# AutoGPTQ/AutoGPTQ

Measured on AMD Instinct MI355X. Metric: int4 g128 QuantLinear fwd GB/s + tokens/s, Llama-7B shapes, higher is better.
Workload: dtype f16; 1 GPU; Llama-7B linear shapes (4096->4096 x4, 4096->11008 x2, 11008->4096) x 32 blocks = 224 layers, int4 g128 no act-order, M=1 rows per step, 128 launches/step in one hipGraph (q|k|v and gate|up of a block: one gptq_forward_multi launch each); layers=224, launches=128, parallelism=single

## Files before the change

### autogptq_amd/csrc/capi.hip

```cpp
#include <stdarg.h>
#include <stdio.h>
#include <string.h>

#include <algorithm>
#include <cstdlib>
#include <vector>

#include "common.cuh"
#include "launch.h"
#include "../../include/gptq_mi355x_lab.h"

using namespace gptq;

namespace {

thread_local char g_err[512] = "";

int fail(int code, const char* fmt, ...) {
    va_list ap;
    va_start(ap, fmt);
    vsnprintf(g_err, sizeof(g_err), fmt, ap);
    va_end(ap);
    return code;
}
// ... 1687 lines not shown
    if (e != hipSuccess) return hip_fail(e, "gptq_unprepack_decode launch");
    return GPTQ_OK;
}

int gptq_permute_columns(const void* x, const int32_t* perm, int M, int K, int dtype, void* x_out, void* stream) {
    if (!x || !perm || !x_out) return fail(GPTQ_ERR_NULL, "x/perm/x_out must be non-NULL");
    if (!dtype_ok(dtype)) return fail(GPTQ_ERR_UNSUPPORTED, "unsupported dtype enum %d", dtype);
    if (M <= 0 || K <= 0) return fail(GPTQ_ERR_SHAPE, "M (%d) and K (%d) must be > 0", M, K);
    hipError_t e = launch_permute_columns(x, perm, M, K, dtype, x_out, (hipStream_t)stream);
    if (e != hipSuccess) return hip_fail(e, "gptq_permute_columns launch");
    return GPTQ_OK;
}

int gptq_describe_plan(const gptq_layer_t* L, int M, const gptq_tuning_t* tune, char* out, size_t out_bytes) {
    if (!out || out_bytes == 0) return fail(GPTQ_ERR_NULL, "out must be non-NULL");
    out[0] = 0;
    int rc = check_layer(L);
    if (rc) return rc;
    if (M <= 0) return fail(GPTQ_ERR_SHAPE, "M must be > 0, got %d", M);
    if (tune && (tune->path == 2 || tune->path == 4)) return fail(GPTQ_ERR_UNSUPPORTED, "tuning.path = %d was retired in round 6", tune->path);
    if (tiled_pair_call(L, M, tune)) {
        const gptq_layer_t* one[1] = {L};
        const TiledPlan tp = plan_tiled(one, 1, M, tune);
        snprintf(out, out_bytes, "path=gemv kernel=strips ln=4 waves=%d u=%d ksplit=%d mt=%d strips=%d pair=1 perm=0 epilogue=fused", tp.waves, tp.u, tp.ksplit, tp.mt,
                 tp.strips_total);
        return GPTQ_OK;
    }
    const bool unfused_epilogue = L->epilogue != GPTQ_EPI_NONE && !fused_epilogue_ok(L, M, tune);
    gptq_layer_t Lc = *L;
    gptq_tuning_t local;
    if (unfused_epilogue) {
        Lc.epilogue = GPTQ_EPI_NONE;
        tune = inner_tuning(L, M, tune, &local);
    }
    gptq_layer_t Pseq;
    const gptq_layer_t* one_t[1] = {&Lc};
    if (!unfused_epilogue && Lc.epilogue == GPTQ_EPI_NONE && want_tiled(one_t, 1, M, tune)) {
        const TiledPlan tp = plan_tiled(one_t, 1, M, tune);
        snprintf(out, out_bytes, "path=gemv kernel=strips ln=4 waves=%d u=%d ksplit=%d mt=%d strips=%d pair=0 perm=0 epilogue=none", tp.waves, tp.u, tp.ksplit, tp.mt,
                 tp.strips_total);
    } else if (!unfused_epilogue && want_stream_seq(L, M, tune, &Pseq)) {
        const gptq_layer_t* one[1] = {&Pseq};
        const StreamPlan sp = plan_stream(one, 1, M, nullptr);
        snprintf(out, out_bytes, "path=gemv kernel=stream ln=%d waves=%d u=%d ksplit=%d mt=%d strips=%d pair=0 perm=2 epilogue=none", sp.ln, sp.waves,
                 sp.u, sp.ksplit, sp.mt, sp.strips_total);
    } else if (want_stream(&Lc, M, tune)) {
        const gptq_layer_t* one[1] = {&Lc};
        const StreamPlan sp = plan_stream(one, 1, M, tune);
        snprintf(out, out_bytes, "path=gemv kernel=stream ln=%d waves=%d u=%d ksplit=%d mt=%d strips=%d pair=0 perm=0 epilogue=none", sp.ln, sp.waves,
                 sp.u, sp.ksplit, sp.mt, sp.strips_total);
    } else if (want_gemm(&Lc, M, tune)) {
        const GemmPlan g = plan_gemm(Lc, M, tune);
        const char* kern = g.f32 ? "f32_mfma" : g.rows ? "rows" : g.panel ? "panel" : g.wsk ? "wide_sk" : g.wide ? (g.wide_tiled ? "wide_copy" : "wide") : g.mid ? "mid" : (g.stream64 ? "stream64" : (g.strip16 ? "strip16" : (g.skinny ? "skinny64" : "tiled")));
        snprintf(out, out_bytes, "path=gemm kernel=%s mt=%d bk=%d kg=%d ksplit=%d tiles=%dx%d tail=%d tail_slices=%d perm=%d dma=%d waves=%d u=%d epilogue=%s", kern, g.mt, g.bk,
                 g.kg == 2 ? 2 : 1, g.ksplit, g.nbm, g.nbn, g.tail, g.tail ? (1 << g.tail_lg) : 1, g.use_seq ? 1 : 0, (g.glds || g.stream64 || g.mid) ? 1 : 0, g.waves, g.u,
                 unfused_epilogue ? "separate" : "none");
    } else {
        const GemvPlan v = plan_gemv(Lc, M, tune);
        const char* kern = v.mfma ? "mfma" : (v.mfmag ? "mfma_generic" : "generic");
        snprintf(out, out_bytes, "path=gemv kernel=%s ln=%d waves=%d u=%d ksplit=%d mt=%d strips=%d pair=%d perm=%d epilogue=%s%s", kern, v.ln,
                 v.waves, v.u, v.ksplit, v.mt, v.strips, v.pair ? 1 : 0, v.xperm ? 2 : (v.use_seq ? 1 : 0),
                 v.pair ? "fused" : (unfused_epilogue ? "separate" : "none"), v.magic ? " deq=magic" : "");
    }
// ... 110 lines not shown
```

### autogptq_amd/csrc/gemv_tiled.hip

```cpp
#include "gemv_tiled_kernel.cuh"

namespace gptq {

hipError_t launch_tiled_act(const TiledPlan& pl, const TiledParams& p, int dtype, hipStream_t st);
hipError_t init_gemv_tiled_act_device();
hipError_t launch_tiled_peer(const TiledPlan& pl, const TiledParams& p, int dtype, hipStream_t st);
hipError_t init_gemv_tiled_peer_device();
hipError_t launch_tiled_pair(const TiledPlan& pl, const TiledParams& p, int dtype, hipStream_t st);
hipError_t init_gemv_tiled_pair_device();
hipError_t launch_tiled_multi(const TiledPlan& pl, const TiledParams& p, int dtype, hipStream_t st);
hipError_t init_gemv_tiled_multi_device();

int tiled_max_waves(int u, int nstr) { return (u == 2 || nstr == 4) ? 16 : 8; }
static int tiled_kpl(int bits) { return bits == 8 ? 16 : 32; }
static int tiled_chunk_bytes(int bits) { return bits == 3 ? 768 : (bits == 2 ? 512 : 1024); }
static int tiled_rec_bytes(int bits) { return bits == 8 ? 64 : 48; }

static bool tiled_pair_layer(const gptq_layer_t& L) { return L.epilogue == GPTQ_EPI_SILU_MUL && L.g_idx == nullptr && L.N % (2 * GPTQ_STRIP_COLS) == 0; }

bool tiled_layer_ok(const gptq_layer_t& L) {
    if (!L.qweight_tiled || !L.qconst_tiled || L.tiled_cols != GPTQ_STRIP_COLS || (L.epilogue != GPTQ_EPI_NONE && !tiled_pair_layer(L))) return false;
    if (L.bits != 4 && L.bits != 8 && L.bits != 3 && L.bits != 2) return false;
    if (L.bits == 2 && L.epilogue != GPTQ_EPI_NONE) return false;
    if (L.g_idx != nullptr && !(L.perm && L.qweight_seq)) return false;
    if (L.dtype != GPTQ_F16 && L.dtype != GPTQ_BF16) return false;
    if (L.K % 32 || L.N % GPTQ_STRIP_COLS) return false;
    const int kpl = tiled_kpl(L.bits);
    const int gu = L.group_size / kpl;
    return L.group_size % kpl == 0 && (L.group_size >= L.K || (gu & (gu - 1)) == 0);
}

size_t tiled_weight_bytes(const gptq_layer_t& L) {
    const int cke = 4 * tiled_kpl(L.bits);
    return (size_t)((L.K + cke - 1) / cke) * tiled_chunk_bytes(L.bits) * (size_t)(L.N / GPTQ_STRIP_COLS);
}
size_t tiled_const_bytes(const gptq_layer_t& L) {
// ... 71 lines not shown
    if (tune && tune->waves && tune->reserved[0]) {
        waves = tune->waves; u = tune->reserved[0];
    } else {
        const int wgs = strips * pl.ksplit;
        if (wgs <= 256) { waves = 16; u = 2; }
        else if (wgs <= 512) { waves = 8; u = 2; }
        else { waves = 4; u = 4; }
        if (wgs <= 128 && chunks >= 64 && pl.ksplit == 1) { waves = 8; u = 4; }
        if (pl.mt > 4) { waves = 8; u = 4; }
        if (pair && waves == 4) waves = 8;
        if (pair && waves == 8 && u == 4 && (double)((chunks + 15) / 16 * 16) / chunks - (double)((chunks + 7) / 8 * 8) / chunks >= 0.1) u = 2;
        if (nstr > 1) { waves = nstr == 4 ? 16 : 8; u = 4; }
        if (nstr == 2 && pl.mt <= 2 && A.K <= 7168) waves = 4;
        if (nstr == 2 && pl.mt == 4 && waves == 8 && (double)((chunks + 15) / 16 * 16) / chunks - (double)((chunks + 7) / 8 * 8) / chunks >= 0.1) u = 2;
        if (pl.mt == 4 && waves == 4 && !pair && nstr == 1 && ((size_t)160 * 1024 / lds_need(ks, 4)) * 4 < 12) waves = 8;
        const int per = pair ? 2 : nstr;
        while (waves > per && (waves / (2 * per)) * u >= cps) waves /= 2;
    }
    if (pair && (waves & 1)) return pl;
    if (nstr > 1 && pl.mt <= 2 && (waves > 8 || u != 4)) return pl;
    if (nstr > 1 && waves % nstr != 0) return pl;
    if (waves < 1 || waves > 16 || (u != 2 && u != 4)) return pl;
    if (waves > tiled_max_waves(u, nstr)) return pl;
    pl.waves = waves;
    pl.u = u;
    pl.zm2 = A.bits == 4 && A.dtype == GPTQ_BF16 && pl.mt == 2 && (long)strips * pl.ksplit < 1024;
    pl.xstride = cps * cke * 2 + 16;
    pl.lds_bytes = lds_need(pl.ksplit, waves);
    pl.xraw_off = A.g_idx ? (int)((pl.lds_bytes - ((size_t)pl.mt * ((size_t)A.K * 2 + 16) + 16) + 15) & ~(size_t)15) : 0;
    if (pl.lds_bytes > 160 * 1024) return pl;
    pl.partial_bytes = pl.ksplit > 1 ? (size_t)(pl.ksplit - 1) * M * nsum * 8 : 0;
    pl.ok = true;
    return pl;
}

hipError_t launch_tiled(const gptq_layer_t* const* Ls, const TiledPlan& pl, const void* x, void* const* outs, int M, void* ws_header, void* ws_body,
                        hipStream_t st, const gptq_peer_group_t* pg) {
    if (!pl.ok) return hipErrorInvalidValue;
    TiledParams p{};
    if (pg) {
        if (pl.nseg != 1 || pl.mt > 4 || pg->world < 1 || pg->world > GPTQ_PEER_MAX) return hipErrorInvalidValue;
        for (int r = 0; r < pg->world; ++r) {
            p.peer.xbuf[0][r] = (char*)pg->xbuf[0][r];
            p.peer.xbuf[1][r] = (char*)pg->xbuf[1][r];
            p.peer.flags[r] = pg->flags[r];
        }
        p.peer.state = pg->state;
        p.peer.world = pg->world;
        p.peer.rank = pg->rank;
// ... 17 lines not shown
    const gptq_layer_t& A = *Ls[0];
    p.x = x;
    p.gran = (unsigned long long*)ws_body;
    p.epochs = ws_header ? (unsigned*)((char*)ws_header + WS_HEADER_EPOCH_OFFSET) : nullptr;
    p.err = ws_header ? (unsigned*)((char*)ws_header + WS_HEADER_BYTES - WS_HEADER_TAIL_BYTES) + 2 : nullptr;
#ifdef GPTQ_TILED_STAMPS
    if (pl.ksplit == 1) {
        const char* const e = getenv("GPTQ_TILED_STAMPS_PTR");
        p.gran = e ? (unsigned long long*)strtoull(e, nullptr, 0) : nullptr;
    }
#endif
    p.max_spins = 1u << 20;
    p.nseg = pl.nseg; p.M = M; p.K = A.K;
    p.chunks = pl.chunks_total; p.chunks_per_split = pl.chunks_per_split; p.ksplit = pl.ksplit;
    p.gu_shift = A.group_size >= A.K ? 26 : __builtin_ctz((unsigned)(A.group_size / tiled_kpl(A.bits)));
    p.nsum = pl.nsum;
    p.groups = pl.groups;
    p.xstride = pl.xstride;
    p.waves = pl.waves;
    p.xraw_off = pl.xraw_off;
    p.pair_strips = pl.pair ? A.N / (2 * GPTQ_STRIP_COLS) : 0;
    if (pg) {
        if (A.g_idx || A.bits == 2 || (pl.u != 2 && pl.u != 4)) return hipErrorInvalidValue;
        return launch_tiled_peer(pl, p, A.dtype, st);
    }
    if (pl.pair) return (pl.u == 2 || pl.u == 4) ? launch_tiled_pair(pl, p, A.dtype, st) : hipErrorInvalidValue;
    if (pl.nstr > 1) return (pl.u == 2 || pl.u == 4) ? launch_tiled_multi(pl, p, A.dtype, st) : hipErrorInvalidValue;
    if (A.g_idx) return launch_tiled_act(pl, p, A.dtype, st);
    return A.dtype == GPTQ_BF16 ? launch_tiled_bits<bf16, 0>(pl, p, st) : launch_tiled_bits<f16, 0>(pl, p, st);
}

hipError_t init_gemv_tiled_device() {
    hipError_t e = grant_tiled_lds<0>();
    hipError_t e2 = init_gemv_tiled_act_device();
    hipError_t e3 = init_gemv_tiled_peer_device();
    hipError_t e4 = init_gemv_tiled_pair_device();
    hipError_t e5 = init_gemv_tiled_multi_device();
    return e != hipSuccess ? e : (e2 != hipSuccess ? e2 : (e3 != hipSuccess ? e3 : (e4 != hipSuccess ? e4 : e5)));
}

}
```

### autogptq_amd/csrc/gemv_tiled_kernel.cuh

```cuda
#pragma once
#include <cstddef>

#include "gemv_shared.cuh"

namespace gptq {

struct TiledSeg {
    const void* bias;
    void* out;
    int N, col0;
};
struct PeerEpi {
    char* xbuf[2][GPTQ_PEER_MAX];
    unsigned* flags[GPTQ_PEER_MAX];
    unsigned* state;
    int world, rank;
    unsigned row_bytes, col_off_bytes, owners, pad_;
};
struct TiledParams {
    int blk_end[4];
    const void* x;
    int M, K;
    int chunks, chunks_per_split, ksplit, gu_shift, groups, xstride, waves;
    int pair_strips;
// ... 9 lines not shown
    unsigned* err;
    PeerEpi peer;
};
static_assert(offsetof(TiledParams, perm) == 128, "the entry batch of the decode-copy kernel is the first two cache lines of its arguments");

template <int BITS> struct TiledFmt;
template <> struct TiledFmt<4> { static constexpr int WPL = 4, KPL = 32, REC = 48, ZB = 1; };
template <> struct TiledFmt<8> { static constexpr int WPL = 4, KPL = 16, REC = 64, ZB = 2; };
template <> struct TiledFmt<3> { static constexpr int WPL = 3, KPL = 32, REC = 48, ZB = 1; };
template <> struct TiledFmt<2> { static constexpr int WPL = 2, KPL = 32, REC = 48, ZB = 1; };

#ifdef GPTQ_TILED_STAMPS
#define TILED_STAMP(i) (st_[i] = __builtin_amdgcn_s_memtime() | vz_)
#define TILED_STAMPS_OUT() stamps_out()
#define TILED_HOT_END() return
#else
#define TILED_HOT_END() __builtin_amdgcn_endpgm()
#define TILED_STAMP(i) ((void)0)
#define TILED_STAMPS_OUT() ((void)0)
#endif

template <int N_> struct WordsOf { typedef unsigned type __attribute__((ext_vector_type(N_))); };

template <int BITS, int MT, int U, typename T, int MAXW, int XM = 0, int ZM2 = 0>
__global__ void __launch_bounds__(MAXW * 64, MAXW == 16 ? 4 : 2) gemv_tiled_kernel(TiledParams p) {
#ifdef GPTQ_TILED_STAMPS
    unsigned long long st_[9] = {};
    unsigned vz_;
    asm volatile("v_mov_b32 %0, 0" : "=v"(vz_));
    st_[7] = __builtin_amdgcn_s_memrealtime() | vz_;
    TILED_STAMP(0);
    auto stamps_out = [&]() {
        st_[8] = __builtin_amdgcn_s_memrealtime() | vz_;
        unsigned long long* const dbg = p.gran;
        const int b = (int)blockIdx.x, nb = (int)gridDim.x;
        const int slot = b == 0 ? 0 : (b == 1 ? 1 : (b == nb / 2 ? 2 : (b == nb - 1 ? 3 : -1)));
        if (dbg != nullptr && p.ksplit == 1 && slot >= 0 && (threadIdx.x & 63) == 0) {
#pragma unroll
            for (int i = 0; i < 9; ++i) dbg[(slot * 16 + (int)(threadIdx.x >> 6)) * 16 + i] = st_[i];
        }
    };
#endif
    constexpr bool BF = std::is_same_v<T, bf16>;
    constexpr bool ACT = XM == 1, PEER = XM == 3;
    constexpr bool PAIR = XM == 4;
    constexpr bool MULTI = XM == 5 || XM == 6;
    constexpr int NSTR = PAIR ? 2 : (XM == 5 ? 4 : (XM == 6 ? 2 : 1));
    using F = TiledFmt<BITS>;
// ... 65 lines not shown
            "s_mov_b64 %[tq], %[tq1]\n\ts_mov_b64 %[cs], %[cs1]\n\ts_mov_b32 %[sb], %[e0]\n\ts_mov_b32 %[s], 1\n\t"
            "s_cmp_ge_i32 %[i], %[e1]\n\ts_cselect_b64 %[tq], %[tq2], %[tq]\n\ts_cselect_b64 %[cs], %[cs2], %[cs]\n\ts_cselect_b32 %[sb], %[e1], %[sb]\n\ts_cselect_b32 %[s], 2, %[s]\n\t"
            "s_cmp_ge_i32 %[i], %[e2]\n\ts_cselect_b64 %[tq], %[tq3], %[tq]\n\ts_cselect_b64 %[cs], %[cs3], %[cs]\n\ts_cselect_b32 %[sb], %[e2], %[sb]\n\ts_cselect_b32 %[s], 3, %[s]\n"
            "1:"
            : [tq] "+&s"(tqs_), [cs] "+&s"(csts_), [sb] "+&s"(sbase), [s] "+&s"(s)
            : [i] "s"(sidx), [e0] "s"(be0), [e1] "s"(be1), [e2] "s"(be2), [tq1] "s"(hb[1]), [tq2] "s"(hb[2]), [tq3] "s"(hb[3]), [cs1] "s"(hb[5]), [cs2] "s"(hb[6]), [cs3] "s"(hb[7])
            : "scc");
    gchar* const tqs = (gchar*)tqs_;
    gchar* const csts = (gchar*)csts_;
    [[maybe_unused]] const int* const permp = (const int*)perm_;
    const int strip = sidx - sbase;
    const int Wh = NSTR == 4 ? (W >> 2) : (NSTR == 2 ? (W >> 1) : W);
    const int sel = NSTR == 1 ? 0 : (scalar_ge(wave, Wh) + (NSTR == 4 ? scalar_ge(wave, 2 * Wh) + scalar_ge(wave, 3 * Wh) : 0));
    const int wv = NSTR == 1 ? wave : wave - sel * Wh;
    const int strip_w = PAIR ? strip + sel * hstrips : (MULTI ? strip * NSTR + sel : strip);
    char* const xs = smem;
    char* const cs = smem + (size_t)MT * xstride;
    const unsigned crec = (unsigned)G * (unsigned)REC;
    const size_t cpad = ((size_t)crec + 15) & ~(size_t)15;
    float* const red = (float*)(cs + NSTR * cpad);
    gchar* const tb = tqs + (size_t)(unsigned)strip_w * ((unsigned)nchunks * (unsigned)CHB);
    gchar* const cg = csts + (size_t)(unsigned)(MULTI ? strip * NSTR : strip) * crec;
    const unsigned t_lane = (unsigned)lane * (WPL * 4u);
    auto stage_all = [&]() __attribute__((always_inline)) {
        const unsigned xs_lds = (unsigned)(size_t)(__attribute__((address_space(3))) char*)xs, cs_lds = (unsigned)(size_t)(__attribute__((address_space(3))) char*)cs;
        const int w64 = wave * 64, step = W * 64;
        gchar* xrow[MT];
        unsigned xdst[MT];
        if constexpr (XM == 0 || XM == 3 || XM == 4 || MULTI) {
#pragma unroll
            for (int m = 0; m < MT; ++m) {
                xrow[m] = xg + (unsigned)((m == 0 ? 0 : min(m, Mrows - 1)) * K + kbeg) * 2u;
                xdst[m] = xs_lds + m * xstride;
            }
            stage_rows<MT, false>(xrow, xdst, tid, w64, step, (kend - kbeg) >> 3);
        } else if constexpr (ACT) {
#pragma unroll
            for (int m = 0; m < MT; ++m) {
                xrow[m] = xg + (unsigned)((m == 0 ? 0 : min(m, Mrows - 1)) * K) * 2u;
                xdst[m] = xs_lds + (unsigned)xraw_off + m * (K * 2 + 16);
            }
            stage_rows<MT, false>(xrow, xdst, tid, w64, step, K >> 3);
        }
        const int cpieces = (int)(crec >> 4) * (MULTI ? NSTR : 1);
        if constexpr (PAIR) {
            gchar* const crow[2] = {cg, cg + (size_t)(unsigned)hstrips * crec};
// ... 90 lines not shown
        }
        __syncthreads();
    };
    auto x_sums = [&]() {
        const int prow = (kend - kbeg) >> 3, total = prow * MT;
        for (int i0 = 0; i0 < total; i0 += W * 64) {
            const int idx = i0 + tid;
            const bool ok = idx < total;
            int m = 0, pc = ok ? idx : 0;
            if constexpr (MT > 1) { m = pc / prow; pc -= m * prow; }
            u32x4 v = {0u, 0u, 0u, 0u};
            if (ok) v = *(const u32x4*)(xs + (size_t)m * xstride + (size_t)pc * 16);
            float sm = 0.f;
#pragma unroll
            for (int i = 0; i < 4; ++i) sm += __builtin_bit_cast(float, v[i] << 16) + __builtin_bit_cast(float, v[i] & 0xffff0000u);
            sm += __shfl_xor(sm, 1, 64);
            if constexpr (NX == 4) sm += __shfl_xor(sm, 2, 64);
            if (ok && (pc & (NX - 1)) == 0) xe[(pc / NX) * 4 + m] = sm;
        }
        __syncthreads();
    };
    const char* const xl = xs + (size_t)min(lane & 3, MT - 1) * xstride + kb * (KPL * 2);
    const char* const xl2 = xs + (size_t)min(4 + (lane & 3), MT - 1) * xstride + kb * (KPL * 2);
    float acc[MT];
#pragma unroll
    for (int m = 0; m < MT; ++m) acc[m] = 0.f;
    const f16x2 k960 = {(f16)960.f, (f16)960.f}, k896 = {(f16)896.f, (f16)896.f}, k1008 = {(f16)1008.f, (f16)1008.f};
    const f16x2 r16 = {(f16)0.0625f, (f16)0.0625f}, r8 = {(f16)0.125f, (f16)0.125f}, r64 = {(f16)0.015625f, (f16)0.015625f};
    const f16x2 k768 = {(f16)768.f, (f16)768.f}, k1020 = {(f16)1020.f, (f16)1020.f}, r4 = {(f16)0.25f, (f16)0.25f}, r256 = {(f16)0.00390625f, (f16)0.00390625f};
    auto bits_of = [&](f16x2 hv) -> unsigned {
        if constexpr (BF && !XC) {
            const bf16x2 o = {(bf16)(float)hv[0], (bf16)(float)hv[1]};
            return __builtin_bit_cast(unsigned, o);
        } else {
            return __builtin_bit_cast(unsigned, hv);
        }
    };
    constexpr int E = MT * 16, NE = (MULTI ? NSTR : 1) * E;
    const int n_t = (MULTI ? strip * NSTR + tid / E : strip) * 16 + (tid & 15);
    float bv0 = 0.f, bv1 = 0.f;
    typedef __attribute__((address_space(1))) T gT;
    int N = 0;
    const void* biasp = nullptr;
    void* outp = nullptr;
    auto seg_request = [&]() __attribute__((always_inline)) {
        int sl = s;
        asm volatile("" : "+s"(sl) : : "memory");
        N = p.seg[sl].N; biasp = p.seg[sl].bias; outp = p.seg[sl].out;
    };
    auto seg_pin = [&]() __attribute__((always_inline)) { asm volatile("" : "+s"(N), "+s"(biasp), "+s"(outp)); };
    bool staged = false;
    auto wload = [&](int c) __attribute__((always_inline)) -> qvec {
        return __builtin_nontemporal_load((const __attribute__((address_space(1))) qvec*)(tb + ((unsigned)min(c, ce - 1) * (unsigned)CHB + t_lane)));
    };
    auto first_pass = [&]() __attribute__((always_inline)) {
        TILED_STAMP(1);
        seg_request();
#ifdef GPTQ_TILED_WEIGHTS_FIRST
        stage_all();
        asm volatile("s_waitcnt vmcnt(0)" ::: "memory");
#else
        asm volatile("s_waitcnt vmcnt(%0)" ::"n"(U) : "memory");
#endif
        if constexpr (ACT) {
            __syncthreads();
            x_gather();
        }
        __syncthreads();
        if constexpr (XC) x_to_f16();
        if constexpr (XS) x_sums();
        seg_pin();
        if (biasp != nullptr && tid < NE && n_t < (PAIR ? N >> 1 : N)) {
            bv0 = DType<T>::to_f32(((const gT*)biasp)[n_t]);
            if constexpr (PAIR) bv1 = DType<T>::to_f32(((const gT*)biasp)[n_t + (N >> 1)]);
        }
        TILED_STAMP(2);
        staged = true;
    };
    auto chunk = [&](const int cj, const qvec qv) __attribute__((always_inline)) {
        const int cc = min(cj, ce - 1);
        const int k0 = cc * CKE + kb * KPL;
        const bool live = (cj < ce) && (k0 < K);
        const int g = min(k0 >> LKPL >> gshift, G - 1);
        const char* cp = cs + (NSTR > 1 ? (size_t)sel * cpad : (size_t)0) + g * REC;
        const unsigned short sraw = *(const unsigned short*)(cp + col * 2);
        unsigned z;
        if constexpr (F::ZB == 1) z = *(const unsigned char*)(cp + 32 + col);
        else z = *(const unsigned short*)(cp + 32 + col * 2);
        u32x4 xa[NX];
#pragma unroll
        for (int w = 0; w < NX; ++w) xa[w] = *(const u32x4*)(xl + ((unsigned)(cc - cb) * (unsigned)(CKE * 2) + w * 16u));
        u32x4 xb[MT > 4 ? NX : 1];
        if constexpr (MT > 4) {
#pragma unroll
            for (int w = 0; w < NX; ++w) xb[w] = *(const u32x4*)(xl2 + ((unsigned)(cc - cb) * (unsigned)(CKE * 2) + w * 16u));
        }
        const f16x2 c1 = as_f16x2(z * 0x00010001u + 0xE400E400u);
        f32x4 accg = {0.f, 0.f, 0.f, 0.f}, accg2 = {0.f, 0.f, 0.f, 0.f};
        auto mm = [&](int pc, int hf, unsigned b0, unsigned b1) __attribute__((always_inline)) {
            accg = Mma4<MM>::run(u32x2{xa[pc][hf * 2], xa[pc][hf * 2 + 1]}, u32x2{b0, b1}, accg);
            if constexpr (MT > 4) accg2 = Mma4<MM>::run(u32x2{xb[pc][hf * 2], xb[pc][hf * 2 + 1]}, u32x2{b0, b1}, accg2);
        };
        if constexpr (BITS == 4 && ZM) {
            unsigned mgz;
            asm("v_mov_b32 %0, %1" : "=v"(mgz) : "n"(BF ? 0x43004300 : 0x64006400));
            const unsigned nz = z * 0x00010001u + (BF ? 0xC300C300u : 0xE400E400u);
            f32x4 accz = {0.f, 0.f, 0.f, 0.f};
#pragma unroll
            for (int w = 0; w < 4; ++w) {
                const unsigned qw = qv[w];
                mm(w, 0, (qw & m_lo) | mgz, ((qw >> 4) & m_lo) | mgz);
                mm(w, 1, ((qw >> 8) & m_lo) | mgz, ((qw >> 12) & m_lo) | mgz);
                accz = Mma4<MM>::run(u32x2{xa[w][0], xa[w][1]}, u32x2{nz, nz}, accz);
                accz = Mma4<MM>::run(u32x2{xa[w][2], xa[w][3]}, u32x2{nz, nz}, accz);
            }
            accg += accz;
        } else if constexpr (BITS == 4 && XS) {
            unsigned magicb;
            asm("v_mov_b32 %0, 0x43004300" : "=v"(magicb));
#pragma unroll
            for (int w = 0; w < 4; ++w) {
                const unsigned qw = qv[w];
                mm(w, 0, (qw & m_lo) | magicb, ((qw >> 4) & m_lo) | magicb);
                mm(w, 1, ((qw >> 8) & m_lo) | magicb, ((qw >> 12) & m_lo) | magicb);
            }
        } else if constexpr (BITS == 4) {
            const f16x2 c2 = c1 + k960;
#pragma unroll
            for (int w = 0; w < 4; ++w) {
                const unsigned qw = qv[w], q8 = qw >> 8;
                const f16x2 h0 = as_f16x2((qw & m_lo) | magic) + c1;
                const f16x2 h1 = as_f16x2((qw & m_hi) | magic) * r16 + c2;
                const f16x2 h2 = as_f16x2((q8 & m_lo) | magic) + c1;
                const f16x2 h3 = as_f16x2((q8 & m_hi) | magic) * r16 + c2;
                mm(w, 0, bits_of(h0), bits_of(h1));
                mm(w, 1, bits_of(h2), bits_of(h3));
            }
        } else if constexpr (BITS == 2) {
            const f16x2 c4 = c1 + k768, c16 = c1 + k960, c64 = c1 + k1008, c256 = c1 + k1020;
#pragma unroll
            for (int w = 0; w < 2; ++w) {
                const unsigned t = qv[w], t10 = t >> 10;
                const unsigned p0 = bits_of(as_f16x2((t & m2a) | magic) + c1);
                const unsigned p1 = bits_of(as_f16x2((t & m2b) | magic) * r4 + c4);
                const unsigned p2 = bits_of(as_f16x2((t & m2c) | magic) * r16 + c16);
                const unsigned p3 = bits_of(as_f16x2((t & m2d) | magic) * r64 + c64);
                const unsigned p4 = bits_of(as_f16x2((t & m2e) | magic) * r256 + c256);
                const unsigned p5 = bits_of(as_f16x2((t10 & m2a) | magic) + c1);
                const unsigned p6 = bits_of(as_f16x2((t10 & m2b) | magic) * r4 + c4);
                const unsigned p7 = bits_of(as_f16x2((t10 & m2c) | magic) * r16 + c16);
                mm(2 * w, 0, p0, p1);
                mm(2 * w, 1, p2, p3);
                mm(2 * w + 1, 0, p4, p5);
// ... 12 lines not shown
            const f16x2 c6 = c1 + k1008;
            unsigned pr[16];
#pragma unroll
            for (int w = 0; w < 3; ++w) {
                const unsigned t = qv[w], t6 = t >> 6;
                pr[5 * w + 0] = bits_of(as_f16x2((t & m3a) | magic) + c1);
                pr[5 * w + 1] = bits_of(as_f16x2((t & m3b) | magic) * r8 + c3);
                pr[5 * w + 2] = bits_of(as_f16x2((t & m3c) | magic) * r64 + c6);
                pr[5 * w + 3] = bits_of(as_f16x2((t6 & m3b) | magic) * r8 + c3);
                pr[5 * w + 4] = bits_of(as_f16x2((t6 & m3c) | magic) * r64 + c6);
            }
            const unsigned e = ((qv[0] >> 15) & 0x00010001u) | ((qv[1] >> 14) & 0x00020002u) | ((qv[2] >> 13) & 0x00040004u);
            pr[15] = bits_of(as_f16x2(e | magic) + c1);
#pragma unroll
            for (int i = 0; i < 8; ++i) mm(i >> 1, i & 1, pr[2 * i], pr[2 * i + 1]);
        }
        unsigned sr_ = sraw;
        asm volatile("" : "+v"(sr_));
        const float sc = DType<T>::to_f32(__builtin_bit_cast(T, (unsigned short)sr_));
        if constexpr (XS) {
            const float* const xv = xe + ((cc - cb) * 4 + kb) * 4;
            const float zc = (float)(128u + z);
#pragma unroll
            for (int m = 0; m < MT; ++m) acc[m] = live ? fmaf(sc, fmaf(-zc, xv[m], accg[m]), acc[m]) : acc[m];
        } else if constexpr (XC) {
            const float* const xi = xe + ((cc - cb) * 4 + kb) * 4;
#pragma unroll
            for (int m = 0; m < MT; ++m) acc[m] = live ? fmaf(sc * xi[m], accg[m], acc[m]) : acc[m];
        } else {
#pragma unroll
            for (int m = 0; m < MT; ++m) acc[m] = live ? fmaf(sc, m < 4 ? accg[m] : accg2[m - 4], acc[m]) : acc[m];
        }
    };
#ifdef GPTQ_TILED_NO_ROLL
    for (int cbase = cb; cbase < ce; cbase += Wh * U) {
        const int c0 = cbase + wv * U;
        qvec q[U];
#pragma unroll
        for (int j = 0; j < U; ++j) q[j] = wload(c0 + j);
        if (!staged) first_pass();
#ifdef GPTQ_TILED_STAMPS
        if (cbase + Wh * U >= ce) { asm volatile("s_waitcnt vmcnt(0)" ::: "memory"); TILED_STAMP(3); }
#endif
#pragma unroll
        for (int j = 0; j < U; ++j) chunk(c0 + j, q[j]);
    }
#else
    if (cb < ce) {
        int c0 = cb + wv * U;
        qvec q[U];
#pragma unroll
        for (int j = 0; j < U; ++j) q[j] = wload(c0 + j);
        first_pass();
        for (int cn = c0 + Wh * U; cn < ce; cn += Wh * U) {
#pragma unroll
            for (int j = 0; j < U; ++j) {
                chunk(c0 + j, q[j]);
                __builtin_amdgcn_sched_barrier(0);
                q[j] = wload(cn + j);
                __builtin_amdgcn_sched_barrier(0);
            }
            c0 = cn;
        }
#ifdef GPTQ_TILED_STAMPS
        asm volatile("s_waitcnt vmcnt(0)" ::: "memory"); TILED_STAMP(3);
#endif
#pragma unroll
        for (int j = 0; j < U; ++j) chunk(c0 + j, q[j]);
    }
#endif
    TILED_STAMP(4);
#pragma unroll
    for (int m = 0; m < MT; ++m) acc[m] = kslot_sum_swap(acc[m]);
    if (__builtin_expect(!staged, 0)) {
        seg_request();
        seg_pin();
        __syncthreads();
    }
    gT* const outg = (gT*)outp;
    if (lane < 16) {
#pragma unroll
        for (int m = 0; m < MT; ++m) red[wave * ES + m * 16 + lane] = acc[m];
    }
    __syncthreads();
    TILED_STAMP(5);
    if constexpr (PAIR) {
        const int NH = N >> 1;
        if (tid < E) {
            const int m = tid >> 4;
            const float* const r = red + tid;
            float s0 = 0.f, s1 = 0.f;
// ... 63 lines not shown
            TILED_HOT_END();
        }
    }
    T* const stage = PEER ? (T*)xs : nullptr;
    const TiledSeg sg{biasp, outp, N, ksplit != 1 ? p.seg[s].col0 : 0};
    stream_finish<16, MT, T, TiledParams, TiledSeg>(p, sg, strip, sidx, ks, N, red, stage);
    if constexpr (PEER) if (ks == 0) {
        const int pworld = p.peer.world;
        __syncthreads();
        const unsigned e = __hip_atomic_load(p.peer.state, __ATOMIC_RELAXED, __HIP_MEMORY_SCOPE_AGENT) + 1u;
        if (tid < pworld * MT * 2) {
            const int r = tid / (MT * 2), m = (tid >> 1) % MT, q = tid & 1;
            if (m < Mrows) {
                const u32x4 v = *(const u32x4*)((const char*)stage + m * 32 + q * 16);
                char* const dst = p.peer.xbuf[e & 1u][r] + (size_t)m * p.peer.row_bytes + p.peer.col_off_bytes + (size_t)strip * 32 + q * 16;
                asm volatile("global_store_dwordx4 %0, %1, off sc0 sc1\n\ts_nop 1" ::"v"(dst), "v"(v) : "memory");
            }
        }
    }
}

template <int U, int XM> constexpr int tiled_maxw() { return (U == 2 || XM == 5) ? 16 : 8; }
int tiled_max_waves(int u, int nstr);
template <int BITS, int MT, int U, typename T, int XM>
static hipError_t launch_tiled_one(const TiledPlan& pl, const TiledParams& p, hipStream_t st) {
    constexpr int MAXW = tiled_maxw<U, XM>();
    if (pl.waves > MAXW) return hipErrorInvalidValue;
    if constexpr (BITS == 4 && MT == 2 && std::is_same_v<T, bf16> && (XM == 0 || XM == 1)) {
        if (pl.zm2) {
            hipLaunchKernelGGL((gemv_tiled_kernel<BITS, MT, U, T, MAXW, XM, 1>), dim3(pl.strips_total * pl.ksplit), dim3(pl.waves * 64), pl.lds_bytes, st, p);
            return hipGetLastError();
        }
    }
    hipLaunchKernelGGL((gemv_tiled_kernel<BITS, MT, U, T, MAXW, XM>), dim3(pl.strips_total * pl.ksplit), dim3(pl.waves * 64), pl.lds_bytes, st, p);
    return hipGetLastError();
}
template <int BITS, int MT, typename T, int XM>
static hipError_t launch_tiled_u(const TiledPlan& pl, const TiledParams& p, hipStream_t st) {
    switch (pl.u) {
        case 2: if constexpr (!(XM == 6 && MT <= 2)) return launch_tiled_one<BITS, MT, 2, T, XM>(pl, p, st); else return hipErrorInvalidValue;
        case 4: return launch_tiled_one<BITS, MT, 4, T, XM>(pl, p, st);
        default: return hipErrorInvalidValue;
    }
}
template <int BITS, typename T, int XM>
static hipError_t launch_tiled_mt(const TiledPlan& pl, const TiledParams& p, hipStream_t st) {
    constexpr bool LOW_OK = XM != 5 && (XM != 6 || BITS == 4);
    if constexpr (!LOW_OK) {
        if (pl.mt != 4 && pl.mt != 8) return hipErrorInvalidValue;
    }
    switch (pl.mt) {
        case 1: if constexpr (LOW_OK) return launch_tiled_u<BITS, 1, T, XM>(pl, p, st); else return hipErrorInvalidValue;
        case 2: if constexpr (LOW_OK) return launch_tiled_u<BITS, 2, T, XM>(pl, p, st); else return hipErrorInvalidValue;
        case 4: return launch_tiled_u<BITS, 4, T, XM>(pl, p, st);
        case 8: if constexpr (XM != 3 && XM != 4 && BITS != 2) return launch_tiled_u<BITS, 8, T, XM>(pl, p, st); else return hipErrorInvalidValue;
        default: return hipErrorInvalidValue;
    }
}
template <typename T, int XM>
static hipError_t launch_tiled_bits(const TiledPlan& pl, const TiledParams& p, hipStream_t st) {
    switch (pl.bits) {
        case 4: return launch_tiled_mt<4, T, XM>(pl, p, st);
        case 8: return launch_tiled_mt<8, T, XM>(pl, p, st);
        case 3: return launch_tiled_mt<3, T, XM>(pl, p, st);
        case 2:
            if constexpr (XM == 0 || XM == 1) { if (pl.mt <= 4) return launch_tiled_mt<2, T, XM>(pl, p, st); }
            return hipErrorInvalidValue;
        default: return hipErrorInvalidValue;
    }
}

template <int XM>
static hipError_t grant_tiled_lds() {
    hipError_t e = hipSuccess;
    auto grant = [&](auto kern) { hipError_t r = hipFuncSetAttribute((const void*)kern, hipFuncAttributeMaxDynamicSharedMemorySize, 160 * 1024); if (e == hipSuccess) e = r; };
    auto grant_mt = [&](auto mt) {
        constexpr int MT = decltype(mt)::value;
        auto grant_u = [&](auto bu, auto uu) {
            constexpr int B = decltype(bu)::value, U = decltype(uu)::value;
            constexpr int MAXW = tiled_maxw<U, XM>();
            grant(gemv_tiled_kernel<B, MT, U, f16, MAXW, XM>); grant(gemv_tiled_kernel<B, MT, U, bf16, MAXW, XM>);
            if constexpr (B == 4 && MT == 2 && (XM == 0 || XM == 1)) grant(gemv_tiled_kernel<B, MT, U, bf16, MAXW, XM, 1>);
        };
        using I2 = std::integral_constant<int, 2>; using I3 = std::integral_constant<int, 3>; using I4 = std::integral_constant<int, 4>; using I8 = std::integral_constant<int, 8>;
        grant_u(I4{}, I2{}); grant_u(I4{}, I4{});
        grant_u(I8{}, I2{}); grant_u(I8{}, I4{}); grant_u(I3{}, I2{}); grant_u(I3{}, I4{});
        if constexpr ((XM == 0 || XM == 1) && MT <= 4) { grant_u(I2{}, I2{}); grant_u(I2{}, I4{}); }
    };
    if constexpr (XM != 5 && XM != 6) { grant_mt(std::integral_constant<int, 1>{}); grant_mt(std::integral_constant<int, 2>{}); }
    if constexpr (XM == 6) {
        grant(gemv_tiled_kernel<4, 1, 4, f16, 8, 6>); grant(gemv_tiled_kernel<4, 1, 4, bf16, 8, 6>);
        grant(gemv_tiled_kernel<4, 2, 4, f16, 8, 6>); grant(gemv_tiled_kernel<4, 2, 4, bf16, 8, 6>);
    }
    grant_mt(std::integral_constant<int, 4>{});
    if constexpr (XM != 3 && XM != 4) grant_mt(std::integral_constant<int, 8>{});
    return e;
}

}
```

### autogptq_amd/csrc/launch.h

```cpp
#pragma once
#include <hip/hip_runtime.h>
#include <stddef.h>
#include "../../include/gptq_mi355x.h"

namespace gptq {

struct GemvPlan {
    int ln, waves, ksplit, strips, mt, mtiles;
    int units_total, units_per_split, chunk_units;
    bool perk, use_seq;
    bool mfma;
    bool mfmag;
    bool magic;
    bool pair;
    bool xperm;
    size_t xperm_bytes;
    int u;
    size_t lds_bytes, workspace_bytes;
};
GemvPlan plan_gemv(const gptq_layer_t& L, int M, const gptq_tuning_t* tune);
hipError_t launch_gemv(const gptq_layer_t& L, const GemvPlan& pl, const void* x, void* out, int M,
                       void* workspace, hipStream_t st);

struct MidPlan {
// ... 86 lines not shown
    size_t partial_bytes;
};
StreamPlan plan_stream(const gptq_layer_t* const* layers, int n, int M, const gptq_tuning_t* tune);
hipError_t launch_stream(const gptq_layer_t* const* layers, const StreamPlan& pl, const void* x, void* const* outs, int M,
                         void* ws_header, void* ws_body, hipStream_t st);
struct Stream64Plan {
    bool ok;
    bool pays;
    int nseg, mt, waves, u, ksplit, ksteps_total, ksteps_per_split, strips_total, nsum;
    size_t lds_bytes;
    size_t partial_bytes;
};
Stream64Plan plan_stream64(const gptq_layer_t* const* layers, int n, int M, const gptq_tuning_t* tune);
hipError_t launch_stream64(const gptq_layer_t* const* layers, const Stream64Plan& pl, const void* x, void* const* outs, int M,
                           void* ws_header, void* partial, const uint32_t* qweight_override, hipStream_t st);
struct TiledPlan {
    bool ok;
    int nstr;
    bool pair;
    int nseg, bits, waves, u, mt, ksplit, chunks_total, chunks_per_split, strips_total, nsum, groups, xstride, xraw_off;
    size_t lds_bytes;
    size_t partial_bytes;
    bool zm2;
};
bool tiled_layer_ok(const gptq_layer_t& L);
TiledPlan plan_tiled(const gptq_layer_t* const* layers, int n, int M, const gptq_tuning_t* tune);
hipError_t launch_tiled(const gptq_layer_t* const* layers, const TiledPlan& pl, const void* x, void* const* outs, int M, void* ws_header, void* ws_body,
                        hipStream_t st, const gptq_peer_group_t* pg = nullptr);
hipError_t init_gemv_tiled_device();
size_t tiled_weight_bytes(const gptq_layer_t& L);
size_t tiled_const_bytes(const gptq_layer_t& L);
hipError_t launch_prepack_decode(const uint32_t* qweight, const uint32_t* qzeros, const void* scales, int K, int N, int bits, int group_size, int zero_mode,
                                 uint32_t* tiled_out, void* const_out, hipStream_t st);
hipError_t launch_unprepack_decode(const uint32_t* tiled, int K, int N, int bits, uint32_t* qweight_out, hipStream_t st);
bool stream_preferred(const gptq_layer_t& L, int M);
bool multi_preferred(const gptq_layer_t* const* layers, int n, int M);
hipError_t launch_silu_mul2(const void* g, const void* u, void* out, size_t total, int dtype, hipStream_t st);
bool silu_mul2_permute_ok(int K, int dtype);
hipError_t launch_silu_mul2_permute(const void* g, const void* u, const int32_t* perm, int M, int K, int dtype, void* out, hipStream_t st);
hipError_t init_mlp_device();
bool wide_gemm_ok(const gptq_layer_t& L, int M, bool use_seq, bool xslot_glds);
hipError_t launch_gemm_wide(const gptq_layer_t& L, const uint32_t* qweight, const void* x, void* out, int M, bool glds, hipStream_t st, bool tiled = false);
bool wide_sk_ok(const gptq_layer_t& L, int M);
bool wide_sk_pays(const gptq_layer_t& L, int M);
WideSkGeom wide_sk_geom(const gptq_layer_t& L, int M);
hipError_t launch_gemm_wide_sk(const gptq_layer_t& L, const void* x, void* out, int M, void* ws_header, void* slots, hipStream_t st);
// ... 149 lines not shown
```

### include/gptq_mi355x_lab.h

```cpp
#ifndef GPTQ_MI355X_LAB_H
#define GPTQ_MI355X_LAB_H

#define GPTQ_LAB_DEPTH 0

#define GPTQ_LAB_OPT 1
#define GPTQ_LAB_OPT_FIELD_DECODE 1
#define GPTQ_LAB_OPT_MID_XREG 1
#define GPTQ_LAB_OPT_MID_GRANULES 3
#define GPTQ_LAB_OPT_GEMM_BK32 32

#define GPTQ_LAB_GEMM_KERNEL 2
#define GPTQ_LAB_GEMM_SKINNY 1
#define GPTQ_LAB_GEMM_TILED 2
#define GPTQ_LAB_GEMM_STRIP16 3
#define GPTQ_LAB_GEMM_STREAM64 4
#define GPTQ_LAB_GEMM_MID 5

#define GPTQ_LAB_GEMM_VARIANT 3
#define GPTQ_LAB_VARIANT_PLAIN_LOOP 1
#define GPTQ_LAB_VARIANT_SETPRIO 2
#define GPTQ_LAB_VARIANT_CROSS_STEP 3
#define GPTQ_LAB_VARIANT_REG_STAGED_X 5
#define GPTQ_LAB_VARIANT_ONE_K_GROUP 6
#define GPTQ_LAB_VARIANT_TWO_K_GROUPS 7
#define GPTQ_LAB_VARIANT_TAIL_ON 40
#define GPTQ_LAB_VARIANT_TAIL_OFF 41
#define GPTQ_LAB_VARIANT_TAIL_NO_LIMIT 42
#define GPTQ_LAB_VARIANT_WIDE_OFF 44
#define GPTQ_LAB_VARIANT_WIDE_ON 45
#define GPTQ_LAB_VARIANT_WIDE_ROWS 46
#define GPTQ_LAB_VARIANT_WIDE_ROWS_ON 47
#define GPTQ_LAB_VARIANT_WIDE_SK_ON 48
#define GPTQ_LAB_VARIANT_WIDE_SK_OFF 49
#define GPTQ_LAB_VARIANT_ROWS_ON 50
#define GPTQ_LAB_VARIANT_ROWS_OFF 51
#define GPTQ_LAB_VARIANT_PANEL_ON 52
#define GPTQ_LAB_VARIANT_PANEL_OFF 53
#define GPTQ_LAB_VARIANT_MLP_TWO_PASSES 54

#endif
```

Before: 3809 GB/s.

## Add aligned-K specialization of tiled int4 GEMV with scalar base addressing and steady-state loop

Adds an 'aligned' variant of the tiled strip GEMV kernel for 4-bit layers whose K is a multiple of the chunk size (MT=1 single-strip, or multi-strip MT<=2 with U=4). In the steady-state loop it skips the per-chunk clamping and liveness checks, reads LDS through address-space-3 pointers with a running x offset, and computes the weight base address in scalar registers through readfirstlane. The aim is to cut VALU and address-arithmetic overhead in the memory-bound inner loop. It also adds compile-time ablation hooks and a tuning variant that forces the general path, and it doubles the kernel instantiations for those forms, which increases code size.

```diff
diff --git a/autogptq_amd/csrc/capi.hip b/autogptq_amd/csrc/capi.hip
--- a/autogptq_amd/csrc/capi.hip
+++ b/autogptq_amd/csrc/capi.hip
@@ -1733,8 +1733,8 @@
     if (tiled_pair_call(L, M, tune)) {
         const gptq_layer_t* one[1] = {L};
         const TiledPlan tp = plan_tiled(one, 1, M, tune);
-        snprintf(out, out_bytes, "path=gemv kernel=strips ln=4 waves=%d u=%d ksplit=%d mt=%d strips=%d pair=1 perm=0 epilogue=fused", tp.waves, tp.u, tp.ksplit, tp.mt,
-                 tp.strips_total);
+        snprintf(out, out_bytes, "path=gemv kernel=strips ln=4 waves=%d u=%d ksplit=%d mt=%d strips=%d pair=1 perm=0 epilogue=fused aligned=%d", tp.waves, tp.u, tp.ksplit, tp.mt,
+                 tp.strips_total, tp.aligned ? 1 : 0);
         return GPTQ_OK;
     }
     const bool unfused_epilogue = L->epilogue != GPTQ_EPI_NONE && !fused_epilogue_ok(L, M, tune);
@@ -1748,8 +1748,8 @@
     const gptq_layer_t* one_t[1] = {&Lc};
     if (!unfused_epilogue && Lc.epilogue == GPTQ_EPI_NONE && want_tiled(one_t, 1, M, tune)) {
         const TiledPlan tp = plan_tiled(one_t, 1, M, tune);
-        snprintf(out, out_bytes, "path=gemv kernel=strips ln=4 waves=%d u=%d ksplit=%d mt=%d strips=%d pair=0 perm=0 epilogue=none", tp.waves, tp.u, tp.ksplit, tp.mt,
-                 tp.strips_total);
+        snprintf(out, out_bytes, "path=gemv kernel=strips ln=4 waves=%d u=%d ksplit=%d mt=%d strips=%d pair=0 perm=0 epilogue=none aligned=%d", tp.waves, tp.u, tp.ksplit, tp.mt,
+                 tp.strips_total, tp.aligned ? 1 : 0);
     } else if (!unfused_epilogue && want_stream_seq(L, M, tune, &Pseq)) {
         const gptq_layer_t* one[1] = {&Pseq};
         const StreamPlan sp = plan_stream(one, 1, M, nullptr);
diff --git a/autogptq_amd/csrc/gemv_tiled.hip b/autogptq_amd/csrc/gemv_tiled.hip
--- a/autogptq_amd/csrc/gemv_tiled.hip
+++ b/autogptq_amd/csrc/gemv_tiled.hip
@@ -1,4 +1,5 @@
 #include "gemv_tiled_kernel.cuh"
+#include "../../include/gptq_mi355x_lab.h"
 
 namespace gptq {
 
@@ -12,6 +13,7 @@
 hipError_t init_gemv_tiled_multi_device();
 
 int tiled_max_waves(int u, int nstr) { return (u == 2 || nstr == 4) ? 16 : 8; }
+bool tiled_has_aligned(int bits, int mt, int u, int nstr) { return bits == 4 && ((nstr == 1 && mt == 1) || (nstr == 2 && mt <= 2 && u == 4)); }
 static int tiled_kpl(int bits) { return bits == 8 ? 16 : 32; }
 static int tiled_chunk_bytes(int bits) { return bits == 3 ? 768 : (bits == 2 ? 512 : 1024); }
 static int tiled_rec_bytes(int bits) { return bits == 8 ? 64 : 48; }
@@ -129,9 +131,12 @@
     if (nstr > 1 && waves % nstr != 0) return pl;
     if (waves < 1 || waves > 16 || (u != 2 && u != 4)) return pl;
     if (waves > tiled_max_waves(u, nstr)) return pl;
+    if (nstr == 4 && u == 2 && A.bits != 4) return pl;
     pl.waves = waves;
     pl.u = u;
     pl.zm2 = A.bits == 4 && A.dtype == GPTQ_BF16 && pl.mt == 2 && (long)strips * pl.ksplit < 1024;
+    pl.aligned = A.K % cke == 0 && !A.g_idx && !pair && tiled_has_aligned(A.bits, pl.mt, u, nstr) &&
+                 !(tune && tune->reserved[GPTQ_LAB_GEMM_VARIANT] == GPTQ_LAB_VARIANT_TILED_GENERAL);
     pl.xstride = cps * cke * 2 + 16;
     pl.lds_bytes = lds_need(pl.ksplit, waves);
     pl.xraw_off = A.g_idx ? (int)((pl.lds_bytes - ((size_t)pl.mt * ((size_t)A.K * 2 + 16) + 16) + 15) & ~(size_t)15) : 0;
@@ -195,7 +200,9 @@
     p.pair_strips = pl.pair ? A.N / (2 * GPTQ_STRIP_COLS) : 0;
     if (pg) {
         if (A.g_idx || A.bits == 2 || (pl.u != 2 && pl.u != 4)) return hipErrorInvalidValue;
-        return launch_tiled_peer(pl, p, A.dtype, st);
+        TiledPlan plg = pl;
+        plg.aligned = false;
+        return launch_tiled_peer(plg, p, A.dtype, st);
     }
     if (pl.pair) return (pl.u == 2 || pl.u == 4) ? launch_tiled_pair(pl, p, A.dtype, st) : hipErrorInvalidValue;
     if (pl.nstr > 1) return (pl.u == 2 || pl.u == 4) ? launch_tiled_multi(pl, p, A.dtype, st) : hipErrorInvalidValue;
diff --git a/autogptq_amd/csrc/gemv_tiled_kernel.cuh b/autogptq_amd/csrc/gemv_tiled_kernel.cuh
--- a/autogptq_amd/csrc/gemv_tiled_kernel.cuh
+++ b/autogptq_amd/csrc/gemv_tiled_kernel.cuh
@@ -55,8 +55,15 @@
 
 template <int N_> struct WordsOf { typedef unsigned type __attribute__((ext_vector_type(N_))); };
 
-template <int BITS, int MT, int U, typename T, int MAXW, int XM = 0, int ZM2 = 0>
+template <int BITS, int MT, int U, typename T, int MAXW, int XM = 0, int FL = 0>
 __global__ void __launch_bounds__(MAXW * 64, MAXW == 16 ? 4 : 2) gemv_tiled_kernel(TiledParams p) {
+    constexpr int ZM2 = FL & 1;
+#ifdef GPTQ_TILED_ABL
+    constexpr int ABL = GPTQ_TILED_ABL;
+#else
+    constexpr int ABL = 0;
+#endif
+    constexpr bool AL = (FL & 2) != 0 || (ABL & 1) != 0;
 #ifdef GPTQ_TILED_STAMPS
     unsigned long long st_[9] = {};
     unsigned vz_;
@@ -168,6 +175,7 @@
     gchar* const tb = tqs + (size_t)(unsigned)strip_w * ((unsigned)nchunks * (unsigned)CHB);
     gchar* const cg = csts + (size_t)(unsigned)(MULTI ? strip * NSTR : strip) * crec;
     const unsigned t_lane = (unsigned)lane * (WPL * 4u);
+    [[maybe_unused]] unsigned tlv = t_lane;
     auto stage_all = [&]() __attribute__((always_inline)) {
         const unsigned xs_lds = (unsigned)(size_t)(__attribute__((address_space(3))) char*)xs, cs_lds = (unsigned)(size_t)(__attribute__((address_space(3))) char*)cs;
         const int w64 = wave * 64, step = W * 64;
@@ -304,6 +312,15 @@
     };
     const char* const xl = xs + (size_t)min(lane & 3, MT - 1) * xstride + kb * (KPL * 2);
     const char* const xl2 = xs + (size_t)min(4 + (lane & 3), MT - 1) * xstride + kb * (KPL * 2);
+    typedef __attribute__((address_space(3))) const char lchar;
+    [[maybe_unused]] lchar* const cl = (lchar*)cs + ((NSTR > 1 ? (unsigned)sel * (unsigned)cpad : 0u) + (unsigned)(kb >> gshift) * (unsigned)REC);
+    [[maybe_unused]] lchar* const sl = cl + col * 2;
+    [[maybe_unused]] lchar* const zl = cl + 32 + col * F::ZB;
+    [[maybe_unused]] lchar* const xll = (lchar*)xl;
+    [[maybe_unused]] lchar* const xll2 = (lchar*)xl2;
+    [[maybe_unused]] unsigned xpass = 0u;
+    [[maybe_unused]] unsigned abl_x = 0u;
+    if constexpr ((ABL & 4) != 0) asm("v_mov_b32 %0, 0x3c003c00" : "=v"(abl_x));
     float acc[MT];
 #pragma unroll
     for (int m = 0; m < MT; ++m) acc[m] = 0.f;
@@ -333,7 +350,14 @@
     auto seg_pin = [&]() __attribute__((always_inline)) { asm volatile("" : "+s"(N), "+s"(biasp), "+s"(outp)); };
     bool staged = false;
     auto wload = [&](int c) __attribute__((always_inline)) -> qvec {
-        return __builtin_nontemporal_load((const __attribute__((address_space(1))) qvec*)(tb + ((unsigned)min(c, ce - 1) * (unsigned)CHB + t_lane)));
+        if constexpr (AL) {
+            const unsigned long long sb0 = (unsigned long long)tb + (unsigned long long)((unsigned)min(c, ce - 1) * (unsigned)CHB);
+            const unsigned long long sb = ((unsigned long long)(unsigned)__builtin_amdgcn_readfirstlane((int)(sb0 >> 32)) << 32) | (unsigned)__builtin_amdgcn_readfirstlane((int)(unsigned)sb0);
+            asm volatile("" : "+v"(tlv));
+            return __builtin_nontemporal_load((const __attribute__((address_space(1))) qvec*)((gchar*)sb + tlv));
+        } else {
+            return __builtin_nontemporal_load((const __attribute__((address_space(1))) qvec*)(tb + ((unsigned)min(c, ce - 1) * (unsigned)CHB + t_lane)));
+        }
     };
     auto first_pass = [&]() __attribute__((always_inline)) {
         TILED_STAMP(1);
@@ -359,27 +383,53 @@
         TILED_STAMP(2);
         staged = true;
     };
-    auto chunk = [&](const int cj, const qvec qv) __attribute__((always_inline)) {
-        const int cc = min(cj, ce - 1);
-        const int k0 = cc * CKE + kb * KPL;
-        const bool live = (cj < ce) && (k0 < K);
-        const int g = min(k0 >> LKPL >> gshift, G - 1);
-        const char* cp = cs + (NSTR > 1 ? (size_t)sel * cpad : (size_t)0) + g * REC;
-        const unsigned short sraw = *(const unsigned short*)(cp + col * 2);
+    auto chunk = [&](auto steady_c, const int cj, [[maybe_unused]] const int j, const qvec qv) __attribute__((always_inline)) {
+        constexpr bool STEADY = AL && decltype(steady_c)::value;
+        const int cc = STEADY ? cj : min(cj, ce - 1);
+        bool live;
+        unsigned short sraw;
         unsigned z;
-        if constexpr (F::ZB == 1) z = *(const unsigned char*)(cp + 32 + col);
-        else z = *(const unsigned short*)(cp + 32 + col * 2);
         u32x4 xa[NX];
-#pragma unroll
-        for (int w = 0; w < NX; ++w) xa[w] = *(const u32x4*)(xl + ((unsigned)(cc - cb) * (unsigned)(CKE * 2) + w * 16u));
         u32x4 xb[MT > 4 ? NX : 1];
-        if constexpr (MT > 4) {
-#pragma unroll
-            for (int w = 0; w < NX; ++w) xb[w] = *(const u32x4*)(xl2 + ((unsigned)(cc - cb) * (unsigned)(CKE * 2) + w * 16u));
+        if constexpr (AL) {
+            live = cj < ce;
+            const unsigned go = (unsigned)((cc * 4) >> gshift) * (unsigned)REC;
+            sraw = *(const __attribute__((address_space(3))) unsigned short*)(sl + go);
+            if constexpr (F::ZB == 1) z = *(const __attribute__((address_space(3))) unsigned char*)(zl + go);
+            else z = *(const __attribute__((address_space(3))) unsigned short*)(zl + go);
+            typedef __attribute__((address_space(3))) const u32x4 lx4;
+            const unsigned xo = STEADY ? xpass + (unsigned)j * (unsigned)(CKE * 2) : (unsigned)(cc - cb) * (unsigned)(CKE * 2);
+            lchar* const xp = STEADY ? (lchar*)(size_t)xo : xll + xo;
+#pragma unroll
+            for (int w = 0; w < NX; ++w) xa[w] = *(lx4*)(xp + w * 16u);
+            if constexpr (MT > 4) {
+                lchar* const xp2 = xp + (xll2 - xll);
+#pragma unroll
+                for (int w = 0; w < NX; ++w) xb[w] = *(lx4*)(xp2 + w * 16u);
+            }
+        } else {
+            const int k0 = cc * CKE + kb * KPL;
+            live = (cj < ce) && (k0 < K);
+            const int g = min(k0 >> LKPL >> gshift, G - 1);
+            const char* cp = cs + (NSTR > 1 ? (size_t)sel * cpad : (size_t)0) + g * REC;
+            sraw = *(const unsigned short*)(cp + col * 2);
+            if constexpr (F::ZB == 1) z = *(const unsigned char*)(cp + 32 + col);
+            else z = *(const unsigned short*)(cp + 32 + col * 2);
+#pragma unroll
+            for (int w = 0; w < NX; ++w) xa[w] = *(const u32x4*)(xl + ((unsigned)(cc - cb) * (unsigned)(CKE * 2) + w * 16u));
+            if constexpr (MT > 4) {
+#pragma unroll
+                for (int w = 0; w < NX; ++w) xb[w] = *(const u32x4*)(xl2 + ((unsigned)(cc - cb) * (unsigned)(CKE * 2) + w * 16u));
+            }
+        }
+        if constexpr ((ABL & 4) != 0) {
+#pragma unroll
+            for (int w = 0; w < NX; ++w) xa[w] = u32x4{abl_x, abl_x, abl_x, abl_x};
         }
         const f16x2 c1 = as_f16x2(z * 0x00010001u + 0xE400E400u);
         f32x4 accg = {0.f, 0.f, 0.f, 0.f}, accg2 = {0.f, 0.f, 0.f, 0.f};
         auto mm = [&](int pc, int hf, unsigned b0, unsigned b1) __attribute__((always_inline)) {
+            if constexpr ((ABL & 8) != 0) { asm volatile("" ::"v"(b0), "v"(b1), "v"(xa[pc][hf * 2]), "v"(xa[pc][hf * 2 + 1])); return; }
             accg = Mma4<MM>::run(u32x2{xa[pc][hf * 2], xa[pc][hf * 2 + 1]}, u32x2{b0, b1}, accg);
             if constexpr (MT > 4) accg2 = Mma4<MM>::run(u32x2{xb[pc][hf * 2], xb[pc][hf * 2 + 1]}, u32x2{b0, b1}, accg2);
         };
@@ -411,6 +461,7 @@
 #pragma unroll
             for (int w = 0; w < 4; ++w) {
                 const unsigned qw = qv[w], q8 = qw >> 8;
+                if constexpr ((ABL & 2) != 0) { mm(w, 0, qw, qw); mm(w, 1, qw, qw); continue; }
                 const f16x2 h0 = as_f16x2((qw & m_lo) | magic) + c1;
                 const f16x2 h1 = as_f16x2((qw & m_hi) | magic) * r16 + c2;
                 const f16x2 h2 = as_f16x2((q8 & m_lo) | magic) + c1;
@@ -469,14 +520,14 @@
             const float* const xv = xe + ((cc - cb) * 4 + kb) * 4;
             const float zc = (float)(128u + z);
 #pragma unroll
-            for (int m = 0; m < MT; ++m) acc[m] = live ? fmaf(sc, fmaf(-zc, xv[m], accg[m]), acc[m]) : acc[m];
+            for (int m = 0; m < MT; ++m) acc[m] = (STEADY || live) ? fmaf(sc, fmaf(-zc, xv[m], accg[m]), acc[m]) : acc[m];
         } else if constexpr (XC) {
             const float* const xi = xe + ((cc - cb) * 4 + kb) * 4;
 #pragma unroll
-            for (int m = 0; m < MT; ++m) acc[m] = live ? fmaf(sc * xi[m], accg[m], acc[m]) : acc[m];
+            for (int m = 0; m < MT; ++m) acc[m] = (STEADY || live) ? fmaf(sc * xi[m], accg[m], acc[m]) : acc[m];
         } else {
 #pragma unroll
-            for (int m = 0; m < MT; ++m) acc[m] = live ? fmaf(sc, m < 4 ? accg[m] : accg2[m - 4], acc[m]) : acc[m];
+            for (int m = 0; m < MT; ++m) acc[m] = (STEADY || live) ? fmaf(sc, m < 4 ? accg[m] : accg2[m - 4], acc[m]) : acc[m];
         }
     };
 #ifdef GPTQ_TILED_NO_ROLL
@@ -490,7 +541,7 @@
         if (cbase + Wh * U >= ce) { asm volatile("s_waitcnt vmcnt(0)" ::: "memory"); TILED_STAMP(3); }
 #endif
 #pragma unroll
-        for (int j = 0; j < U; ++j) chunk(c0 + j, q[j]);
+        for (int j = 0; j < U; ++j) chunk(std::false_type{}, c0 + j, j, q[j]);
     }
 #else
     if (cb < ce) {
@@ -499,21 +550,23 @@
 #pragma unroll
         for (int j = 0; j < U; ++j) q[j] = wload(c0 + j);
         first_pass();
+        if constexpr (AL) { xpass = (unsigned)(size_t)xll + (unsigned)(c0 - cb) * (unsigned)(CKE * 2); asm volatile("" : "+v"(xpass)); }
         for (int cn = c0 + Wh * U; cn < ce; cn += Wh * U) {
 #pragma unroll
             for (int j = 0; j < U; ++j) {
-                chunk(c0 + j, q[j]);
+                chunk(std::true_type{}, c0 + j, j, q[j]);
                 __builtin_amdgcn_sched_barrier(0);
                 q[j] = wload(cn + j);
                 __builtin_amdgcn_sched_barrier(0);
             }
             c0 = cn;
+            if constexpr (AL) { xpass += (unsigned)(Wh * U) * (unsigned)(CKE * 2); asm volatile("" : "+v"(xpass)); }
         }
 #ifdef GPTQ_TILED_STAMPS
         asm volatile("s_waitcnt vmcnt(0)" ::: "memory"); TILED_STAMP(3);
 #endif
 #pragma unroll
-        for (int j = 0; j < U; ++j) chunk(c0 + j, q[j]);
+        for (int j = 0; j < U; ++j) chunk(std::false_type{}, c0 + j, j, q[j]);
     }
 #endif
     TILED_STAMP(4);
@@ -623,10 +676,20 @@
 
 template <int U, int XM> constexpr int tiled_maxw() { return (U == 2 || XM == 5) ? 16 : 8; }
 int tiled_max_waves(int u, int nstr);
+template <int BITS, int MT, int U, int XM> constexpr bool tiled_aligned_form() { return BITS == 4 && ((XM == 0 && MT == 1) || (XM == 6 && MT <= 2 && U == 4)); }
+bool tiled_has_aligned(int bits, int mt, int u, int nstr);
 template <int BITS, int MT, int U, typename T, int XM>
 static hipError_t launch_tiled_one(const TiledPlan& pl, const TiledParams& p, hipStream_t st) {
     constexpr int MAXW = tiled_maxw<U, XM>();
     if (pl.waves > MAXW) return hipErrorInvalidValue;
+    if constexpr (tiled_aligned_form<BITS, MT, U, XM>()) {
+        if (pl.aligned) {
+            hipLaunchKernelGGL((gemv_tiled_kernel<BITS, MT, U, T, MAXW, XM, 2>), dim3(pl.strips_total * pl.ksplit), dim3(pl.waves * 64), pl.lds_bytes, st, p);
+            return hipGetLastError();
+        }
+    } else if (pl.aligned) {
+        return hipErrorInvalidValue;
+    }
     if constexpr (BITS == 4 && MT == 2 && std::is_same_v<T, bf16> && (XM == 0 || XM == 1)) {
         if (pl.zm2) {
             hipLaunchKernelGGL((gemv_tiled_kernel<BITS, MT, U, T, MAXW, XM, 1>), dim3(pl.strips_total * pl.ksplit), dim3(pl.waves * 64), pl.lds_bytes, st, p);
@@ -639,7 +702,7 @@
 template <int BITS, int MT, typename T, int XM>
 static hipError_t launch_tiled_u(const TiledPlan& pl, const TiledParams& p, hipStream_t st) {
     switch (pl.u) {
-        case 2: if constexpr (!(XM == 6 && MT <= 2)) return launch_tiled_one<BITS, MT, 2, T, XM>(pl, p, st); else return hipErrorInvalidValue;
+        case 2: if constexpr (!(XM == 6 && MT <= 2) && !(XM == 5 && BITS != 4)) return launch_tiled_one<BITS, MT, 2, T, XM>(pl, p, st); else return hipErrorInvalidValue;
         case 4: return launch_tiled_one<BITS, MT, 4, T, XM>(pl, p, st);
         default: return hipErrorInvalidValue;
     }
@@ -680,7 +743,8 @@
         auto grant_u = [&](auto bu, auto uu) {
             constexpr int B = decltype(bu)::value, U = decltype(uu)::value;
             constexpr int MAXW = tiled_maxw<U, XM>();
-            grant(gemv_tiled_kernel<B, MT, U, f16, MAXW, XM>); grant(gemv_tiled_kernel<B, MT, U, bf16, MAXW, XM>);
+            if constexpr (!(XM == 5 && B != 4 && U == 2)) { grant(gemv_tiled_kernel<B, MT, U, f16, MAXW, XM>); grant(gemv_tiled_kernel<B, MT, U, bf16, MAXW, XM>); }
+            if constexpr (tiled_aligned_form<B, MT, U, XM>()) { grant(gemv_tiled_kernel<B, MT, U, f16, MAXW, XM, 2>); grant(gemv_tiled_kernel<B, MT, U, bf16, MAXW, XM, 2>); }
             if constexpr (B == 4 && MT == 2 && (XM == 0 || XM == 1)) grant(gemv_tiled_kernel<B, MT, U, bf16, MAXW, XM, 1>);
         };
         using I2 = std::integral_constant<int, 2>; using I3 = std::integral_constant<int, 3>; using I4 = std::integral_constant<int, 4>; using I8 = std::integral_constant<int, 8>;
@@ -692,6 +756,8 @@
     if constexpr (XM == 6) {
         grant(gemv_tiled_kernel<4, 1, 4, f16, 8, 6>); grant(gemv_tiled_kernel<4, 1, 4, bf16, 8, 6>);
         grant(gemv_tiled_kernel<4, 2, 4, f16, 8, 6>); grant(gemv_tiled_kernel<4, 2, 4, bf16, 8, 6>);
+        grant(gemv_tiled_kernel<4, 1, 4, f16, 8, 6, 2>); grant(gemv_tiled_kernel<4, 1, 4, bf16, 8, 6, 2>);
+        grant(gemv_tiled_kernel<4, 2, 4, f16, 8, 6, 2>); grant(gemv_tiled_kernel<4, 2, 4, bf16, 8, 6, 2>);
     }
     grant_mt(std::integral_constant<int, 4>{});
     if constexpr (XM != 3 && XM != 4) grant_mt(std::integral_constant<int, 8>{});
diff --git a/autogptq_amd/csrc/launch.h b/autogptq_amd/csrc/launch.h
--- a/autogptq_amd/csrc/launch.h
+++ b/autogptq_amd/csrc/launch.h
@@ -132,6 +132,7 @@
     size_t lds_bytes;
     size_t partial_bytes;
     bool zm2;
+    bool aligned;
 };
 bool tiled_layer_ok(const gptq_layer_t& L);
 TiledPlan plan_tiled(const gptq_layer_t* const* layers, int n, int M, const gptq_tuning_t* tune);
diff --git a/include/gptq_mi355x_lab.h b/include/gptq_mi355x_lab.h
--- a/include/gptq_mi355x_lab.h
+++ b/include/gptq_mi355x_lab.h
@@ -37,5 +37,6 @@
 #define GPTQ_LAB_VARIANT_PANEL_ON 52
 #define GPTQ_LAB_VARIANT_PANEL_OFF 53
 #define GPTQ_LAB_VARIANT_MLP_TWO_PASSES 54
+#define GPTQ_LAB_VARIANT_TILED_GENERAL 60
 
 #endif
```

Result: faster. 3890 GB/s, median of 6 (+2.1%).
